# UCF-CRCV/TeD-SPAD

Measured on AMD Instinct MI355X. Metric: clips/sec (16x224^2 I3D features), higher is better.
Workload: dtype f16; 1 GPU; cfg2 dali_extraction path: largei3d extract_features, 225 clip times x 10 crops = 2250 clip-forwards of 3x16x224x224 per GPU per step, random-init weights; global_batch=375, parallelism=clip-sharded x1 + RCCL all-gather of (T,10,F) features

## Files before the change

### ted_spad_amd/csrc/conv_flat.hip

```cpp
#include "conv_common.h"

namespace tedspad {
namespace {

__device__ uint4 g_zero16f;

constexpr int FL_BM = 256;
constexpr int FL_WSTAGE = 64 * BK * 2;

struct FlatGeo {
    int W, H, R, NP, ntaps;
};

template <typename T>
__global__ __launch_bounds__(256) void conv_flat_kernel(const ConvKP p, const FlatGeo g) {
    constexpr int NT = 256, WS = 3;
    extern __shared__ __attribute__((aligned(16))) unsigned char dsm[];
    const int tid = threadIdx.x, lane = tid & 63;
    const int wave = __builtin_amdgcn_readfirstlane(tid >> 6);
    const int tile = xcd_remap(blockIdx.x, gridDim.x);
    const int q0 = tile * FL_BM;
    const int S = (g.NP + 1) * 8;
    const int Sr = (S + 63) / 64 * 64;
    const int halo_bytes = Sr * 16;
    unsigned char *wring = dsm + halo_bytes;
    const unsigned lds0 = (unsigned)(uintptr_t)(lptr_t)dsm;
    const uint16_t *zero = reinterpret_cast<const uint16_t *>(&g_zero16f);

    const int rsub = wave * 8 + (lane >> 3);
    const int kc = (lane & 7) ^ ((4 * (wave & 1) + (lane >> 4)) & 7);
    const uint16_t *wsrc = p.w + (size_t)rsub * p.Kpad + kc * 8;
    auto issue_w = [&](int kt, int slot) {
        const unsigned dst = lds0 + halo_bytes + slot * FL_WSTAGE + wave * 8 * (BK * 2);
        lds_dma16(wsrc + kt * BK, dst);
        lds_dma16(wsrc + (size_t)32 * p.Kpad + kt * BK, dst + 32 * (BK * 2));
    };
    issue_w(0, 0);
    const int NH = (Sr + NT - 1) / NT;
    for (int i = 0; i < NH; ++i) {
        if (i * NT + wave * 64 >= Sr) break;
        const int s = i * NT + tid;
        const int pos = s >> 3, cs = s & 7;
        const int q = q0 - g.R + pos;
        const bool ok = pos < g.NP && (unsigned)q < (unsigned)p.M;
        const uint16_t *src = ok ? p.x + (size_t)q * p.ldx + ((cs ^ ((pos >> 1) & 7)) << 3) : zero;
        lds_dma16(src, lds0 + (i * NT + wave * 64) * 16);
    }
    if (g.ntaps > 1) issue_w(1, 1);

    const int l31 = lane & 31, lh = lane >> 5;
    const int swz = (l31 >> 1) & 7;
    int pj[2];
    unsigned vmask[2];
#pragma unroll
    for (int b = 0; b < 2; ++b) {
        const int j = wave * 64 + b * 32 + l31;
        pj[b] = j;
        const int q = q0 + j;
        unsigned mk = 0;
        if (q < p.M) {
            const int r1 = q / g.W, w = q - r1 * g.W;
            const int h = r1 % g.H;
            for (int dh = 0; dh < p.kh; ++dh)
                for (int dw = 0; dw < p.kw; ++dw)
                    if ((unsigned)(h + dh - p.ph) < (unsigned)g.H && (unsigned)(w + dw - p.pw) < (unsigned)g.W) mk |= 1u << (dh * p.kw + dw);
        }
        vmask[b] = mk;
    }
    f32x16 acc[2][2];
#pragma unroll
    for (int a = 0; a < 2; ++a)
#pragma unroll
        for (int b = 0; b < 2; ++b)
#pragma unroll
            for (int r = 0; r < 16; ++r) acc[a][b][r] = 0.f;

    if (g.ntaps > 1) wait_vmcnt<2>(); else wait_vmcnt<0>();
    __builtin_amdgcn_s_barrier();
    asm volatile("" ::: "memory");
    int dh = 0, dw = 0;
    for (int kt = 0; kt < g.ntaps; ++kt) {
        const int delta = dh * g.W + dw;
        unsigned xoff[2], xswz[2];
#pragma unroll
        for (int b = 0; b < 2; ++b) {
            const int pos = ((vmask[b] >> kt) & 1u) ? pj[b] + delta : g.NP;
            xoff[b] = (unsigned)pos * 128u;
            xswz[b] = (unsigned)(pos >> 1) & 7u;
        }
        const uint4 fa00 = *reinterpret_cast<const uint4 *>(dsm + xoff[0] + (((unsigned)lh ^ xswz[0]) << 4));
        const uint4 fa01 = *reinterpret_cast<const uint4 *>(dsm + xoff[1] + (((unsigned)lh ^ xswz[1]) << 4));
        if (kt + 1 < g.ntaps) wait_vmcnt<2>(); else wait_vmcnt<0>();
        __builtin_amdgcn_s_barrier();
        asm volatile("" ::: "memory");
        if (kt + 2 < g.ntaps) issue_w(kt + 2, (kt + 2) % WS);
        const uint16_t *Wt = reinterpret_cast<const uint16_t *>(wring + (kt % WS) * FL_WSTAGE) + l31 * BK;
        {
            const unsigned c = (unsigned)lh;
            const uint4 fw0 = *reinterpret_cast<const uint4 *>(Wt + ((c ^ swz) << 3)), fw1 = *reinterpret_cast<const uint4 *>(Wt + 32 * BK + ((c ^ swz) << 3));
            acc[0][0] = T::mfma(fw0, fa00, acc[0][0]);
            acc[0][1] = T::mfma(fw0, fa01, acc[0][1]);
            acc[1][0] = T::mfma(fw1, fa00, acc[1][0]);
            acc[1][1] = T::mfma(fw1, fa01, acc[1][1]);
        }
#pragma unroll
        for (int ks = 1; ks < 4; ++ks) {
            const unsigned c = (unsigned)((ks << 1) | lh);
            uint4 fa[2], fw[2];
#pragma unroll
            for (int b = 0; b < 2; ++b) fa[b] = *reinterpret_cast<const uint4 *>(dsm + xoff[b] + ((c ^ xswz[b]) << 4));
#pragma unroll
            for (int a = 0; a < 2; ++a) fw[a] = *reinterpret_cast<const uint4 *>(Wt + a * 32 * BK + ((c ^ swz) << 3));
#pragma unroll
            for (int a = 0; a < 2; ++a)
#pragma unroll
                for (int b = 0; b < 2; ++b) acc[a][b] = T::mfma(fw[a], fa[b], acc[a][b]);
        }
        if (++dw == p.kw) { dw = 0; ++dh; }
    }
    __syncthreads();

    constexpr int STG_LD = 64 + 4;
    float *stg = reinterpret_cast<float *>(dsm);
#pragma unroll
    for (int a = 0; a < 2; ++a)
#pragma unroll
        for (int b = 0; b < 2; ++b) {
            const int ml = wave * 64 + b * 32 + l31;
#pragma unroll
            for (int qd = 0; qd < 4; ++qd) {
                f32x4 v = {acc[a][b][4 * qd], acc[a][b][4 * qd + 1], acc[a][b][4 * qd + 2], acc[a][b][4 * qd + 3]};
                *reinterpret_cast<f32x4 *>(stg + ml * STG_LD + a * 32 + 8 * qd + 4 * lh) = v;
            }
        }
    __syncthreads();
    const int cc = tid & 7, r0 = tid >> 3;
    const int nch = cc * 8;
    if (nch >= p.Cout) return;
    float sc[8], sf[8];
#pragma unroll
    for (int i = 0; i < 8; ++i) { sc[i] = p.scale[nch + i]; sf[i] = p.shift[nch + i]; }
#pragma unroll
    for (int it = 0; it < FL_BM / 32; ++it) {
        const int r = r0 + it * 32;
        const size_t m = (size_t)q0 + r;
        if (m >= (size_t)p.M) continue;
        const f32x4 v0 = *reinterpret_cast<const f32x4 *>(stg + r * STG_LD + nch);
        const f32x4 v1 = *reinterpret_cast<const f32x4 *>(stg + r * STG_LD + nch + 4);
        float v[8];
#pragma unroll
        for (int i = 0; i < 4; ++i) { v[i] = v0[i] * sc[i] + sf[i]; v[i + 4] = v1[i] * sc[i + 4] + sf[i + 4]; }
        if (p.res) {
            float rr[8];
            unpack8<T>(*reinterpret_cast<const uint4 *>(p.res + m * p.ldres + nch), rr);
#pragma unroll
            for (int i = 0; i < 8; ++i) v[i] += rr[i];
        }
        if (p.relu) {
#pragma unroll
            for (int i = 0; i < 8; ++i) v[i] = __builtin_fmaxf(v[i], 0.f);
        }
        *reinterpret_cast<uint4 *>(p.y + m * p.ldy + nch) = pack8_lim<T>(v, p.sat);
    }
}

template <typename T>
int32_t launch_flat_t(const ConvKP &p, hipStream_t s) {
    FlatGeo g;
    g.W = p.Wi; g.H = p.Hi; g.R = p.ph * p.Wi + p.pw; g.ntaps = p.kh * p.kw;
    g.NP = FL_BM + (p.kh - 1) * p.Wi + (p.kw - 1);
    const int S = (g.NP + 1) * 8;
    const int main_bytes = (S + 63) / 64 * 64 * 16 + 3 * FL_WSTAGE;
    const int stage_bytes = FL_BM * (64 + 4) * 4;
    const int lds = main_bytes > stage_bytes ? main_bytes : stage_bytes;
    if (lds > 160 * 1024) {
        set_error("tedspad_conv_fwd: flat-halo config: halo does not fit LDS (%d bytes)", lds);
        return TEDSPAD_EINVAL;
    }
    static thread_local int attr_set[2] = {0, 0};
    auto kfn = conv_flat_kernel<T>;
    if (!attr_set[T::kDtype]) {
        if (hipFuncSetAttribute((const void *)kfn, hipFuncAttributeMaxDynamicSharedMemorySize, 160 * 1024) != hipSuccess) {
            set_error("tedspad_conv_fwd: cannot raise the dynamic LDS limit");
            return TEDSPAD_ELAUNCH;
        }
        attr_set[T::kDtype] = 1;
    }
    const int tiles = (p.M + FL_BM - 1) / FL_BM;
    hipLaunchKernelGGL(kfn, dim3(tiles), dim3(256), lds, s, p, g);
    return check_launch("tedspad_conv_fwd(flat halo)");
}

struct TFlatGeo {
    int T, HW, tiles_s, nchunks, kt, pt;
};

template <typename T_>
__global__ __launch_bounds__(256) void conv_tflat_kernel(const ConvKP p, const TFlatGeo g) {
    constexpr int NT = 256;
    constexpr int NP = 256;
    constexpr int HALO = (NP + 8) * 128;
    extern __shared__ __attribute__((aligned(16))) unsigned char dsm[];
    const int tid = threadIdx.x, lane = tid & 63;
    const int wave = __builtin_amdgcn_readfirstlane(tid >> 6);
    const int tile = xcd_remap(blockIdx.x, gridDim.x);
    const int n = tile / g.tiles_s, s0 = (tile - n * g.tiles_s) * 64;
    unsigned char *wbuf = dsm + HALO;
    const unsigned lds0 = (unsigned)(uintptr_t)(lptr_t)dsm;
    const uint16_t *zero = reinterpret_cast<const uint16_t *>(&g_zero16f);

    const int rsub = wave * 8 + (lane >> 3);
    const int kc = (lane & 7) ^ ((4 * (wave & 1) + (lane >> 4)) & 7);
    const uint16_t *wsrc = p.w + (size_t)rsub * p.Kpad + kc * 8;
    int hsrc[9];
#pragma unroll
    for (int i = 0; i < 9; ++i) {
        const int s = i * NT + tid;
        const int pos = s >> 3, cs = s & 7;
        const int f = pos >> 6, px = pos & 63;
        hsrc[i] = -1;
        if (pos < NP && f < g.T && s0 + px < g.HW) hsrc[i] = (int)((((long)n * g.T + f) * g.HW + s0 + px) * p.ldx) + ((cs ^ ((pos >> 1) & 7)) << 3);
    }
    const int l31 = lane & 31, lh = lane >> 5;
    const int swz = (l31 >> 1) & 7;
    f32x16 acc[2][2];
#pragma unroll
    for (int a = 0; a < 2; ++a)
#pragma unroll
        for (int b = 0; b < 2; ++b)
#pragma unroll
            for (int r = 0; r < 16; ++r) acc[a][b][r] = 0.f;

    for (int ch = 0; ch < g.nchunks; ++ch) {
        if (ch) __builtin_amdgcn_s_barrier();
        asm volatile("" ::: "memory");
#pragma unroll
        for (int i = 0; i < 9; ++i) {
            if (i * NT + wave * 64 >= (NP + 8) * 8) break;
            lds_dma16(hsrc[i] >= 0 ? p.x + hsrc[i] + ch * 64 : zero, lds0 + (i * NT + wave * 64) * 16);
        }
        for (int dt = 0; dt < g.kt; ++dt) {
            const unsigned dst = lds0 + HALO + dt * FL_WSTAGE + wave * 8 * (BK * 2);
            const uint16_t *src = wsrc + dt * p.cin + ch * 64;
            lds_dma16(src, dst);
            lds_dma16(src + (size_t)32 * p.Kpad, dst + 32 * (BK * 2));
        }
        wait_vmcnt<0>();
        __builtin_amdgcn_s_barrier();
        asm volatile("" ::: "memory");
        for (int dt = 0; dt < g.kt; ++dt) {
            const int fin = wave + dt - g.pt;
            if (wave >= g.T || fin < 0 || fin >= g.T) continue;
            const uint16_t *Wt = reinterpret_cast<const uint16_t *>(wbuf + dt * FL_WSTAGE) + l31 * BK;
            unsigned xoff[2], xswz[2];
#pragma unroll
            for (int b = 0; b < 2; ++b) {
                const int pos = fin * 64 + b * 32 + l31;
                xoff[b] = (unsigned)pos * 128u;
                xswz[b] = (unsigned)(pos >> 1) & 7u;
            }
#pragma unroll
            for (int ks = 0; ks < 4; ++ks) {
                const unsigned c = (unsigned)((ks << 1) | lh);
                uint4 fa[2], fw[2];
#pragma unroll
                for (int b = 0; b < 2; ++b) fa[b] = *reinterpret_cast<const uint4 *>(dsm + xoff[b] + ((c ^ xswz[b]) << 4));
#pragma unroll
                for (int a = 0; a < 2; ++a) fw[a] = *reinterpret_cast<const uint4 *>(Wt + a * 32 * BK + ((c ^ swz) << 3));
#pragma unroll
                for (int a = 0; a < 2; ++a)
#pragma unroll
                    for (int b = 0; b < 2; ++b) acc[a][b] = T_::mfma(fw[a], fa[b], acc[a][b]);
            }
        }
    }
    __syncthreads();

    constexpr int STG_LD = 64 + 4;
    float *stg = reinterpret_cast<float *>(dsm);
#pragma unroll
    for (int a = 0; a < 2; ++a)
#pragma unroll
        for (int b = 0; b < 2; ++b) {
            const int ml = wave * 64 + b * 32 + l31;
#pragma unroll
            for (int qd = 0; qd < 4; ++qd) {
                f32x4 v = {acc[a][b][4 * qd], acc[a][b][4 * qd + 1], acc[a][b][4 * qd + 2], acc[a][b][4 * qd + 3]};
                *reinterpret_cast<f32x4 *>(stg + ml * STG_LD + a * 32 + 8 * qd + 4 * lh) = v;
            }
        }
    __syncthreads();
    const int cc = tid & 7, r0 = tid >> 3;
    const int nch = cc * 8;
    if (nch >= p.Cout) return;
    float sc[8], sf[8];
#pragma unroll
    for (int i = 0; i < 8; ++i) { sc[i] = p.scale[nch + i]; sf[i] = p.shift[nch + i]; }
#pragma unroll
    for (int it = 0; it < 8; ++it) {
        const int r = r0 + it * 32;
        const int f = r >> 6, px = r & 63;
        if (f >= g.T || s0 + px >= g.HW) continue;
        const size_t m = ((size_t)n * g.T + f) * g.HW + s0 + px;
        const f32x4 v0 = *reinterpret_cast<const f32x4 *>(stg + r * STG_LD + nch);
        const f32x4 v1 = *reinterpret_cast<const f32x4 *>(stg + r * STG_LD + nch + 4);
        float v[8];
#pragma unroll
        for (int i = 0; i < 4; ++i) { v[i] = v0[i] * sc[i] + sf[i]; v[i + 4] = v1[i] * sc[i + 4] + sf[i + 4]; }
        if (p.res) {
            float rr[8];
            unpack8<T_>(*reinterpret_cast<const uint4 *>(p.res + m * p.ldres + nch), rr);
#pragma unroll
            for (int i = 0; i < 8; ++i) v[i] += rr[i];
        }
        if (p.relu) {
#pragma unroll
            for (int i = 0; i < 8; ++i) v[i] = __builtin_fmaxf(v[i], 0.f);
        }
        *reinterpret_cast<uint4 *>(p.y + m * p.ldy + nch) = pack8_lim<T_>(v, p.sat);
    }
}

template <typename T_>
int32_t launch_tflat_t(const ConvKP &p, int N, int cin, hipStream_t s) {
    TFlatGeo g;
    g.T = p.Ti; g.HW = p.Hi * p.Wi; g.tiles_s = (g.HW + 63) / 64; g.nchunks = cin / 64; g.kt = p.kt; g.pt = p.pt;
    const int main_bytes = (256 + 8) * 128 + p.kt * FL_WSTAGE;
    const int stage_bytes = FL_BM * (64 + 4) * 4;
    const int lds = main_bytes > stage_bytes ? main_bytes : stage_bytes;
    static thread_local int attr_set[2] = {0, 0};
    auto kfn = conv_tflat_kernel<T_>;
    if (!attr_set[T_::kDtype]) {
        if (hipFuncSetAttribute((const void *)kfn, hipFuncAttributeMaxDynamicSharedMemorySize, 160 * 1024) != hipSuccess) {
            set_error("tedspad_conv_fwd: cannot raise the dynamic LDS limit");
            return TEDSPAD_ELAUNCH;
        }
        attr_set[T_::kDtype] = 1;
    }
    hipLaunchKernelGGL(kfn, dim3(N * g.tiles_s), dim3(256), lds, s, p, g);
    return check_launch("tedspad_conv_fwd(temporal flat halo)");
}

}

int32_t launch_conv_flat(int dtype, const ConvKP &p, int cin, hipStream_t s) {
    const bool same = p.To == p.Ti && p.Ho == p.Hi && p.Wo == p.Wi && p.pt == 0 && p.ph < p.kh && p.pw < p.kw;
    if (cin != 64 || p.kt != 1 || p.st != 1 || p.sh != 1 || p.sw != 1 || !same || p.kh * p.kw < 2 || p.kh * p.kw > 32 || p.Cout > 64 ||
        p.Kpad != p.kh * p.kw * 64 || p.mask || p.stats || p.ostrided || p.y32 || p.sigmoid || !p.y) {
        set_error("tedspad_conv_fwd: flat-halo config needs a stride-1 'same' 1 x kh x kw conv with cin = 64, cout <= 64 and the plain epilogue");
        return TEDSPAD_EINVAL;
    }
    return dtype == TEDSPAD_F16 ? launch_flat_t<F16>(p, s) : launch_flat_t<BF16>(p, s);
}

}

namespace tedspad {

int32_t launch_conv_tflat(int dtype, const ConvKP &p, int N, int cin, hipStream_t s) {
    const bool same = p.To == p.Ti && p.Ho == p.Hi && p.Wo == p.Wi && p.ph == 0 && p.pw == 0 && p.pt < p.kt;
    if (cin % 64 != 0 || p.kh != 1 || p.kw != 1 || p.kt < 2 || p.kt > 3 || p.st != 1 || p.sh != 1 || p.sw != 1 || !same || p.Ti > 4 || p.Cout > 64 ||
        p.Kpad != p.kt * cin || p.mask || p.stats || p.ostrided || p.y32 || p.sigmoid || !p.y) {
        set_error("tedspad_conv_fwd: temporal flat-halo config needs a stride-1 'same' kt x 1 x 1 conv (kt 2..3) with cin %% 64 == 0, cout <= 64, T <= 4");
        return TEDSPAD_EINVAL;
    }
    return dtype == TEDSPAD_F16 ? launch_tflat_t<F16>(p, N, cin, s) : launch_tflat_t<BF16>(p, N, cin, s);
}

}
```

Baseline: 25050 clips/s.

## Add persistent pipelined kernel for temporal kt x1x1 flat-halo convolution

Adds a persistent kernel for the temporal conv. It uses 512 threads and launches one workgroup per CU, each looping over a contiguous range of spatial tiles. Halo loads are triple-buffered and weights double-buffered through LDS DMA, so loads for later chunks overlap the MFMA work and epilogue of the current one; weights stay resident when there are at most two channel chunks. It is on by default, with env vars to fall back to the old kernel or override the grid size, and it adds pipeline complexity and relies on correct ordering of wait counts and barriers.

Result: no change. 25040 clips/s (median of 2 runs) (-0.0%).

```diff
diff --git a/ted_spad_amd/csrc/conv_flat.hip b/ted_spad_amd/csrc/conv_flat.hip
--- a/ted_spad_amd/csrc/conv_flat.hip
+++ b/ted_spad_amd/csrc/conv_flat.hip
@@ -1,3 +1,5 @@
+#include <stdlib.h>
+
 #include "conv_common.h"
 
 namespace tedspad {
@@ -341,6 +343,206 @@
     return check_launch("tedspad_conv_fwd(temporal flat halo)");
 }
 
+constexpr int TP_NT = 512;
+constexpr int TP_HSLOT = 256 * 128;
+constexpr int TP_W0 = 3 * TP_HSLOT;
+constexpr int TP_WSLOT = 3 * FL_WSTAGE;
+constexpr int TP_BN0 = TP_W0 + 2 * TP_WSLOT;
+constexpr int TP_LDS = TP_BN0 + 2 * 64 * 4;
+
+__device__ __forceinline__ uint2 load8_opaque(const void *ptr) {
+    typedef unsigned u32x2g __attribute__((ext_vector_type(2)));
+    unsigned long a = reinterpret_cast<unsigned long>(ptr);
+    asm volatile("" : "+v"(a));
+    const u32x2g v = *reinterpret_cast<const __attribute__((address_space(1))) u32x2g *>(a);
+    return make_uint2(v.x, v.y);
+}
+
+struct TPipeGeo {
+    int T, HW, tiles_s, nchunks, pt, tiles;
+};
+
+template <typename T_, int KT>
+__global__ __launch_bounds__(TP_NT) void conv_tflat_pipe_kernel(const ConvKP p, const TPipeGeo g) {
+    extern __shared__ __attribute__((aligned(16))) unsigned char dsm[];
+    const int tid = threadIdx.x, lane = tid & 63;
+    const int wave = __builtin_amdgcn_readfirstlane(tid >> 6);
+    const int fr = wave & 3, hb = wave >> 2;
+    const int nwg = gridDim.x;
+    const int run = xcd_remap(blockIdx.x, nwg);
+    const int t0 = (int)((long)run * g.tiles / nwg), t1 = (int)((long)(run + 1) * g.tiles / nwg);
+    const int nsteps = (t1 - t0) * g.nchunks;
+    if (nsteps <= 0) return;
+    const unsigned lds0 = (unsigned)(uintptr_t)(lptr_t)dsm;
+    const uint16_t *zero = reinterpret_cast<const uint16_t *>(&g_zero16f);
+    float *bn = reinterpret_cast<float *>(dsm + TP_BN0);
+    if (tid < 128) {
+        const int c = tid & 63;
+        bn[tid] = c < p.Cout ? (tid < 64 ? p.scale[c] : p.shift[c]) : 0.f;
+    }
+    __syncthreads();
+
+    const int kc = (lane & 7) ^ ((4 * (wave & 1) + (lane >> 4)) & 7);
+    const uint16_t *wsrc = p.w + (size_t)(wave * 8 + (lane >> 3)) * p.Kpad + kc * 8;
+    auto issue_w = [&](int ch, int slot) {
+#pragma unroll
+        for (int dt = 0; dt < KT; ++dt)
+            lds_dma16(wsrc + dt * p.cin + ch * 64, lds0 + TP_W0 + slot * TP_WSLOT + dt * FL_WSTAGE + wave * 8 * (BK * 2));
+    };
+    long hoff[4];
+    auto h_tile = [&](int tile) {
+        const int n = tile / g.tiles_s, s0 = (tile - n * g.tiles_s) * 64;
+#pragma unroll
+        for (int i = 0; i < 4; ++i) {
+            const int s = i * TP_NT + tid;
+            const int pos = s >> 3, cs = s & 7;
+            const int f = pos >> 6, px = pos & 63;
+            hoff[i] = f < g.T && s0 + px < g.HW ? (((long)n * g.T + f) * g.HW + s0 + px) * p.ldx + ((cs ^ ((pos >> 1) & 7)) << 3) : -1;
+        }
+    };
+    int ptile = t0, pch = 0, pslot = 0;
+    auto issue_h = [&]() {
+#pragma unroll
+        for (int i = 0; i < 4; ++i)
+            lds_dma16(hoff[i] >= 0 ? p.x + hoff[i] + pch * 64 : zero, lds0 + pslot * TP_HSLOT + (i * TP_NT + wave * 64) * 16);
+        pslot = pslot == 2 ? 0 : pslot + 1;
+        if (++pch == g.nchunks) {
+            pch = 0;
+            if (++ptile < t1) h_tile(ptile);
+        }
+    };
+    h_tile(t0);
+    issue_w(0, 0);
+    issue_h();
+    if (nsteps > 1) issue_h();
+
+    const int l31 = lane & 31, lh = lane >> 5;
+    const int swz = (l31 >> 1) & 7;
+    f32x16 acc[2];
+#pragma unroll
+    for (int a = 0; a < 2; ++a)
+#pragma unroll
+        for (int r = 0; r < 16; ++r) acc[a][r] = 0.f;
+
+    auto epilogue = [&](int tile) {
+        if (fr >= g.T) return;
+        const int n = tile / g.tiles_s, s0 = (tile - n * g.tiles_s) * 64;
+        const int px = hb * 32 + l31;
+        const bool ok = s0 + px < g.HW;
+        const size_t m = ((size_t)n * g.T + fr) * g.HW + s0 + px;
+#pragma unroll
+        for (int a = 0; a < 2; ++a) {
+            unsigned d[4][2];
+            uint2 rv[4];
+            if (p.res) {
+#pragma unroll
+                for (int qd = 0; qd < 4; ++qd)
+                    rv[qd] = load8_opaque(ok && a * 32 + 8 * qd < p.Cout ? p.res + m * p.ldres + a * 32 + 8 * qd + 4 * lh : zero);
+            }
+#pragma unroll
+            for (int qd = 0; qd < 4; ++qd) {
+                const int c0 = a * 32 + 8 * qd + 4 * lh;
+                const f32x4 sc = *reinterpret_cast<const f32x4 *>(bn + c0), sf = *reinterpret_cast<const f32x4 *>(bn + 64 + c0);
+                float v[4];
+#pragma unroll
+                for (int i = 0; i < 4; ++i) v[i] = acc[a][4 * qd + i] * sc[i] + sf[i];
+                if (p.res) {
+                    v[0] += T_::to_f32((uint16_t)(rv[qd].x & 0xffffu)); v[1] += T_::to_f32((uint16_t)(rv[qd].x >> 16));
+                    v[2] += T_::to_f32((uint16_t)(rv[qd].y & 0xffffu)); v[3] += T_::to_f32((uint16_t)(rv[qd].y >> 16));
+                }
+                if (p.relu) {
+#pragma unroll
+                    for (int i = 0; i < 4; ++i) v[i] = __builtin_fmaxf(v[i], 0.f);
+                }
+                d[qd][0] = (unsigned)T_::from_f32_lim(v[0], p.sat) | ((unsigned)T_::from_f32_lim(v[1], p.sat) << 16);
+                d[qd][1] = (unsigned)T_::from_f32_lim(v[2], p.sat) | ((unsigned)T_::from_f32_lim(v[3], p.sat) << 16);
+            }
+#pragma unroll
+            for (int q = 0; q < 4; q += 2)
+#pragma unroll
+                for (int h = 0; h < 2; ++h) {
+                    auto sw = __builtin_amdgcn_permlane32_swap(d[q][h], d[q + 1][h], false, false);
+                    d[q][h] = sw[0];
+                    d[q + 1][h] = sw[1];
+                }
+#pragma unroll
+            for (int j = 0; j < 2; ++j) {
+                const int nch = a * 32 + 8 * (2 * j + lh);
+                if (ok && nch < p.Cout) *reinterpret_cast<uint4 *>(p.y + m * p.ldy + nch) = make_uint4(d[2 * j][0], d[2 * j][1], d[2 * j + 1][0], d[2 * j + 1][1]);
+            }
+        }
+    };
+
+    int ctile = t0, cch = 0, hs = 0, ws = 0;
+    const bool wres = g.nchunks <= 2;
+    for (int s = 0; s < nsteps; ++s) {
+        if (s + 1 < nsteps) wait_vmcnt<4>(); else wait_vmcnt<0>();
+        __builtin_amdgcn_s_barrier();
+        asm volatile("" ::: "memory");
+        if (cch == 0 && s > 0) {
+            epilogue(ctile - 1);
+#pragma unroll
+            for (int a = 0; a < 2; ++a)
+#pragma unroll
+                for (int r = 0; r < 16; ++r) acc[a][r] = 0.f;
+        }
+        if (s + 1 < nsteps && (!wres || s + 1 < g.nchunks)) issue_w(cch + 1 == g.nchunks ? 0 : cch + 1, ws ^ 1);
+        if (s + 2 < nsteps) issue_h();
+        const unsigned char *hbuf = dsm + hs * TP_HSLOT;
+        const unsigned char *wbuf = dsm + TP_W0 + (wres ? cch : ws) * TP_WSLOT;
+#pragma unroll
+        for (int dt = 0; dt < KT; ++dt) {
+            const int fin = fr + dt - g.pt;
+            if (fr >= g.T || fin < 0 || fin >= g.T) continue;
+            const uint16_t *Wt = reinterpret_cast<const uint16_t *>(wbuf + dt * FL_WSTAGE) + l31 * BK;
+            const int pos = fin * 64 + hb * 32 + l31;
+            const unsigned xoff = (unsigned)pos * 128u, xswz = (unsigned)(pos >> 1) & 7u;
+#pragma unroll
+            for (int ks = 0; ks < 4; ++ks) {
+                const unsigned c = (unsigned)((ks << 1) | lh);
+                const uint4 fa = *reinterpret_cast<const uint4 *>(hbuf + xoff + ((c ^ xswz) << 4));
+                uint4 fw[2];
+#pragma unroll
+                for (int a = 0; a < 2; ++a) fw[a] = *reinterpret_cast<const uint4 *>(Wt + a * 32 * BK + ((c ^ swz) << 3));
+#pragma unroll
+                for (int a = 0; a < 2; ++a) acc[a] = T_::mfma(fw[a], fa, acc[a]);
+            }
+        }
+        hs = hs == 2 ? 0 : hs + 1;
+        ws ^= 1;
+        if (++cch == g.nchunks) { cch = 0; ++ctile; }
+    }
+    epilogue(t1 - 1);
+}
+
+int g_tflat_cus = 0;
+
+template <typename T_>
+int32_t launch_tflat_pipe_t(const ConvKP &p, int N, int cin, hipStream_t s) {
+    TPipeGeo g;
+    g.T = p.Ti; g.HW = p.Hi * p.Wi; g.tiles_s = (g.HW + 63) / 64; g.nchunks = cin / 64; g.pt = p.pt; g.tiles = N * g.tiles_s;
+    if (!g_tflat_cus) {
+        int dev = 0, n = 0;
+        if (hipGetDevice(&dev) != hipSuccess || hipDeviceGetAttribute(&n, hipDeviceAttributeMultiprocessorCount, dev) != hipSuccess || n <= 0) n = 256;
+        g_tflat_cus = n;
+    }
+    const char *nwg_s = getenv("TEDSPAD_TFLAT_NWG");
+    const int nwg_env = nwg_s ? atoi(nwg_s) : 0;
+    int grid = nwg_env > 0 ? nwg_env : g_tflat_cus;
+    if (grid > g.tiles) grid = g.tiles;
+    static thread_local int attr_set[2][2] = {{0, 0}, {0, 0}};
+    auto kfn = p.kt == 3 ? conv_tflat_pipe_kernel<T_, 3> : conv_tflat_pipe_kernel<T_, 2>;
+    if (!attr_set[T_::kDtype][p.kt - 2]) {
+        if (hipFuncSetAttribute((const void *)kfn, hipFuncAttributeMaxDynamicSharedMemorySize, 160 * 1024) != hipSuccess) {
+            set_error("tedspad_conv_fwd: cannot raise the dynamic LDS limit");
+            return TEDSPAD_ELAUNCH;
+        }
+        attr_set[T_::kDtype][p.kt - 2] = 1;
+    }
+    hipLaunchKernelGGL(kfn, dim3(grid), dim3(TP_NT), TP_LDS, s, p, g);
+    return check_launch("tedspad_conv_fwd(temporal flat halo, pipelined)");
+}
+
 }
 
 int32_t launch_conv_flat(int dtype, const ConvKP &p, int cin, hipStream_t s) {
@@ -364,7 +566,9 @@
         set_error("tedspad_conv_fwd: temporal flat-halo config needs a stride-1 'same' kt x 1 x 1 conv (kt 2..3) with cin %% 64 == 0, cout <= 64, T <= 4");
         return TEDSPAD_EINVAL;
     }
-    return dtype == TEDSPAD_F16 ? launch_tflat_t<F16>(p, N, cin, s) : launch_tflat_t<BF16>(p, N, cin, s);
-}
-
-}
+    const char *pipe_s = getenv("TEDSPAD_TFLAT_PIPE");
+    if (pipe_s && atoi(pipe_s) == 0) return dtype == TEDSPAD_F16 ? launch_tflat_t<F16>(p, N, cin, s) : launch_tflat_t<BF16>(p, N, cin, s);
+    return dtype == TEDSPAD_F16 ? launch_tflat_pipe_t<F16>(p, N, cin, s) : launch_tflat_pipe_t<BF16>(p, N, cin, s);
+}
+
+}
```
